# graphdeco-inria/hierarchical-3d-gaussians

Measured on NVIDIA H100. Metric: train-step images/sec (fwd+bwd) @1080p, 3M Gaussians, SH-3, higher is better.
Workload: dtype f32

## Files before the change

### hierarchical-3d-gaussians_b200/csrc/common.cuh

```cuda
#pragma once
#include <cuda_runtime.h>
#include <stdint.h>
#include <stdio.h>
#include <stdlib.h>
#include "../../include/h3dgs.h"

namespace h3dgs {

constexpr float kNearPlane = 0.2f;
constexpr float kFovClamp = 1.3f;
constexpr float kDilation = 0.3f;
constexpr float kLambdaFloor = 0.1f;
constexpr int kTile = H3DGS_TILE;
constexpr int kTilePixels = kTile * kTile;
constexpr float kAlphaCap = 0.99f;
constexpr float kAlphaSkip = 1.0f / 255.0f;
constexpr float kTStop = 0.0001f;
constexpr float kWEps = 0.0000001f;
constexpr uint32_t kKidsMask = 0xFFFFFu;
constexpr int kClampShift = 20;
constexpr uint32_t kSortedKidsMask = 0xFFFFu;
constexpr int kBlockShift = 16;

struct __align__(16) Record { float4 a, b, c; };
// ... 43 lines not shown
    } while (0)

#define H3_LAUNCHED(name, debug, stream)                                                   \
    do {                                                                                   \
        h3dgs::g_launches++;                                                               \
        cudaError_t e__ = cudaGetLastError();                                              \
        if (e__ == cudaSuccess && (debug)) e__ = cudaStreamSynchronize(stream);            \
        if (e__ != cudaSuccess) {                                                          \
            h3dgs::set_error("kernel %s failed: %s", name, cudaGetErrorString(e__));       \
            return H3DGS_ECUDA;                                                            \
        }                                                                                  \
    } while (0)

int launch_preprocess(const h3dgs_raster_args& a, int32_t* radii, float* depths, uint32_t* tiles_touched,
                      uint8_t* rank_mask, Record* records, uint32_t* tile_count, ScanInfo* info, cudaStream_t s);
int launch_tile_scan(const h3dgs_raster_args& a, const uint32_t* tile_count, uint32_t* ranges, ScanInfo* info,
                     uint32_t cap_entries, uint32_t cap_list, cudaStream_t s);
int launch_tile_binning(const h3dgs_raster_args& a, const int32_t* radii, const float* depths, const Record* records,
                        int64_t D, uint32_t max_count, uint8_t* bin, const BinLayout& bl, const uint32_t* ranges,
                        const ScanInfo* info, uint32_t* tile_count, cudaStream_t s);
int launch_preprocess_color(const h3dgs_raster_args& a, const int32_t* radii, const uint32_t* tiles_touched,
                            Record* records, cudaStream_t s);
int launch_sh_backward(const h3dgs_raster_args& a, const int32_t* radii, const uint8_t* rank_mask, const Record* records,
                       const float* accum, float* dL_dmeans3D, float* dL_dsh, cudaStream_t s);
int launch_scan(const uint32_t* in, uint32_t* out, int n, void* temp, size_t temp_bytes, cudaStream_t s, bool debug);
size_t scan_temp_bytes(int n);
size_t sort_temp_bytes(int64_t n);
int launch_binning(const h3dgs_raster_args& a, const int32_t* radii, const float* depths, const uint32_t* offsets,
                   const Record* records, int64_t D, uint8_t* bin, const BinLayout& bl, uint32_t* ranges,
                   cudaStream_t s);
int launch_render_forward(const h3dgs_raster_args& a, const uint32_t* ranges, const Record* sorted_records,
                          float* out_color, float* out_invdepth, float* final_T, uint32_t* n_contrib,
                          uint32_t* tile_max_contrib, cudaStream_t s);
int launch_render_backward(const h3dgs_raster_args& a, const uint32_t* ranges, const Record* sorted_records,
                           const uint32_t* point_list, const float* final_T, const uint32_t* n_contrib,
                           const uint32_t* tile_max_contrib, const float* dL_dcolor, const float* dL_dinvdepth,
                           float* accum , cudaStream_t s);
int launch_preprocess_backward(const h3dgs_raster_args& a, const int32_t* radii, const uint8_t* rank_mask, const Record* records,
                               const float* accum, float* dL_dmeans3D, float* dL_dmeans2D, float* dL_dsh,
                               float* dL_dcolors, float* dL_dopacities, float* dL_dscales, float* dL_drots,
                               float* dL_dcov3D, cudaStream_t s);

#ifdef __CUDACC__
__device__ __forceinline__ void quad_pixel(int tile_x, int tile_y, int warp, int lane, int& px, int& py0) {
    px = tile_x * kTile + 8 * (warp & 1) + (lane & 7);
    py0 = tile_y * kTile + 8 * (warp >> 1) + 2 * (lane >> 3);
}

__device__ __forceinline__ void group_pixel(int tile_x, int tile_y, int warp, int lane, int& px, int& py0) {
    const int g = lane >> 3, k = lane & 7;
    px = tile_x * kTile + 8 * (warp & 1) + 4 * (g & 1) + (k & 3);
    py0 = tile_y * kTile + 8 * (warp >> 1) + 4 * (g >> 1) + 2 * (k >> 2);
}
inline bool use_group_walk(bool dflt) {
    const char* e = getenv("H3DGS_GROUPWALK");
    return (e && e[0]) ? e[0] != '0' : dflt;
}

#endif

struct PeerPtrs { void* p[H3DGS_MAX_PEERS]; int n; };
inline PeerPtrs peer_ptrs(void* const* src, int n) {
    PeerPtrs r; r.n = n > 1 ? n : 0;
    for (int k = 0; k < H3DGS_MAX_PEERS; k++) r.p[k] = (k < r.n) ? src[k] : nullptr;
    return r;
}
struct RowCycle { int shift, world, rank; };
inline RowCycle row_cycle(const h3dgs_raster_args& a) {
    RowCycle c; c.world = a.peer_count > 1 ? a.peer_count : 0; c.rank = a.shard_index; c.shift = a.grad_cyclic_log2;
    return c;
}
inline int cyclic_local_rows(const RowCycle& c, int P) {
    const int blocks = (P + (1 << c.shift) - 1) >> c.shift;
    return ((blocks + c.world - 1 - c.rank) / c.world) << c.shift;
}
#ifdef __CUDACC__
__device__ __forceinline__ int cyclic_row(const RowCycle& c, int local) {
    return ((((local >> c.shift) * c.world + c.rank)) << c.shift) + (local & ((1 << c.shift) - 1));
}
__device__ __forceinline__ bool cyclic_owned(const RowCycle& c, int row) { return ((row >> c.shift) % c.world) == c.rank; }
#endif

#ifdef __CUDACC__
struct StagePtrs { const float* own; const float* stage; int n, rank; size_t slot_floats; };
template <int NPAIR>
__device__ __forceinline__ void gather_accum_pairs(const StagePtrs& sp, uint32_t mask, int i, int first, float (&out)[2 * NPAIR]) {
#pragma unroll
    for (int k = 0; k < 2 * NPAIR; k++) out[k] = 0.f;
#pragma unroll
    for (int r = 0; r < H3DGS_MAX_PEERS; r++) {
        if (r < sp.n && ((mask >> r) & 1u)) {
            const float* row = (r == sp.rank ? sp.own : sp.stage + (size_t)r * sp.slot_floats) + (size_t)i * 10 + 2 * first;
#pragma unroll
            for (int k = 0; k < NPAIR; k++) {
                const float2 v = __ldcg(reinterpret_cast<const float2*>(row + 2 * k));
                out[2 * k] += v.x; out[2 * k + 1] += v.y;
            }
        }
    }
}
#endif
inline StagePtrs stage_ptrs(const h3dgs_raster_args& a, const float* accum) {
    StagePtrs sp; sp.own = accum; sp.n = a.peer_count > 1 ? a.peer_count : 0; sp.rank = a.shard_index;
    sp.stage = sp.n ? static_cast<const float*>(a.peer_stage[a.shard_index]) : nullptr;
    sp.slot_floats = (size_t)a.P * 10;
    return sp;
// ... 18 lines not shown
```

### hierarchical-3d-gaussians_b200/csrc/pair_math.cuh

```cuda
#pragma once

#ifdef H3_PAIR_HOST_EMU
#include <math.h>
#include <stdint.h>
#define H3_PM_FN static inline
namespace h3dgs {
#ifndef H3_SIMT_EMU
struct float4 { float x, y, z, w; };
constexpr float kAlphaCap = 0.99f;
constexpr float kAlphaSkip = 1.0f / 255.0f;
constexpr float kTStop = 0.0001f;
constexpr uint32_t kSortedKidsMask = 0xFFFFu;
#endif
struct f2 { float lo, hi; };
H3_PM_FN f2 pk(float lo, float hi) { return f2{lo, hi}; }
H3_PM_FN void upk(f2 v, float& lo, float& hi) { lo = v.lo; hi = v.hi; }
H3_PM_FN f2 fma2(f2 a, f2 b, f2 c) { return f2{fmaf(a.lo, b.lo, c.lo), fmaf(a.hi, b.hi, c.hi)}; }
H3_PM_FN f2 mul2(f2 a, f2 b) { return f2{a.lo * b.lo, a.hi * b.hi}; }
H3_PM_FN f2 add2(f2 a, f2 b) { return f2{a.lo + b.lo, a.hi + b.hi}; }
H3_PM_FN f2 sub2(f2 a, f2 b) { return f2{a.lo - b.lo, a.hi - b.hi}; }
H3_PM_FN float fast_exp2(float x) { return exp2f(x); }
H3_PM_FN float fast_log2(float x) { return log2f(x); }
H3_PM_FN float rcp_approx(float x) { return 1.0f / x; }
H3_PM_FN float rsq_approx(float x) { return 1.0f / sqrtf(x); }
#else
#define H3_PM_FN __device__ __forceinline__
namespace h3dgs {
struct f2 { float lo, hi; };
H3_PM_FN f2 pk(float lo, float hi) { return f2{lo, hi}; }
H3_PM_FN void upk(f2 v, float& lo, float& hi) { lo = v.lo; hi = v.hi; }
H3_PM_FN f2 fma2(f2 a, f2 b, f2 c) { return f2{__fmaf_rn(a.lo, b.lo, c.lo), __fmaf_rn(a.hi, b.hi, c.hi)}; }
H3_PM_FN f2 mul2(f2 a, f2 b) { return f2{__fmul_rn(a.lo, b.lo), __fmul_rn(a.hi, b.hi)}; }
H3_PM_FN f2 add2(f2 a, f2 b) { return f2{__fadd_rn(a.lo, b.lo), __fadd_rn(a.hi, b.hi)}; }
H3_PM_FN f2 sub2(f2 a, f2 b) { return f2{__fsub_rn(a.lo, b.lo), __fsub_rn(a.hi, b.hi)}; }
H3_PM_FN float fast_exp2(float x) { float y; asm("ex2.approx.ftz.f32 %0, %1;" : "=f"(y) : "f"(x)); return y; }
H3_PM_FN float fast_log2(float x) { float y; asm("lg2.approx.ftz.f32 %0, %1;" : "=f"(y) : "f"(x)); return y; }
H3_PM_FN float rcp_approx(float x) { float y; asm("rcp.approx.ftz.f32 %0, %1;" : "=f"(y) : "f"(x)); return y; }
H3_PM_FN float rsq_approx(float x) { float y; asm("rsqrt.approx.ftz.f32 %0, %1;" : "=f"(y) : "f"(x)); return y; }
#endif

H3_PM_FN f2 bc(float x) { return pk(x, x); }
H3_PM_FN float lo(f2 v) { float a, b; upk(v, a, b); return a; }
H3_PM_FN float hi(f2 v) { float a, b; upk(v, a, b); return b; }
H3_PM_FN float hsum(f2 v) { float a, b; upk(v, a, b); return a + b; }
H3_PM_FN f2 sel2(bool p0, bool p1, f2 x, f2 y) {
    float x0, x1, y0, y1; upk(x, x0, x1); upk(y, y0, y1);
    return pk(p0 ? x0 : y0, p1 ? x1 : y1);
}
H3_PM_FN f2 ex2_2(f2 v) { float a, b; upk(v, a, b); return pk(fast_exp2(a), fast_exp2(b)); }
H3_PM_FN float fast_rcp(float x) { const float r = rcp_approx(x); return r * (2.0f - x * r); }
H3_PM_FN f2 rcp2(f2 x) {
    float x0, x1; upk(x, x0, x1);
    const f2 r = pk(rcp_approx(x0), rcp_approx(x1));
    return mul2(r, fma2(pk(-x0, -x1), r, bc(2.0f)));
}

H3_PM_FN f2 pair_power(const float4& a, const float4& bb, float dx, f2 nfpy, f2& d) {
    d = add2(bc(a.y), nfpy);
    const float A = (a.z * dx) * (dx * -0.5f), B = -a.w * dx, C = -0.5f * bb.x;
    return fma2(fma2(bc(C), d, bc(B)), d, bc(A));
}
H3_PM_FN void pair_gauss(f2 power, float opacity, f2& G, f2& abase) {
    G = ex2_2(mul2(power, bc(1.4426950408889634f)));
    float a0, a1; upk(mul2(bc(opacity), G), a0, a1);
    abase = pk(fminf(kAlphaCap, a0), fminf(kAlphaCap, a1));
}
template <bool HIER, bool GRAD>
H3_PM_FN void pair_hier_alpha(f2 a, float t, uint32_t k , f2& alpha, f2& dadb) {
    alpha = a; dadb = bc(1.0f);
    if (!HIER) return;
    if (k <= 1u || t >= 1.0f) return;
    const float u = 1.0f - t;
    float a0, a1; upk(a, a0, a1);
    float o0, o1; upk(sub2(bc(1.0f), a), o0, o1);
    if (k == 2u) {
        const f2 r = pk(rsq_approx(o0), rsq_approx(o1));
        const f2 s = mul2(pk(o0, o1), r);
        f2 S = fma2(a, bc(0.02734375f), bc(0.0390625f));
        S = fma2(a, S, bc(0.0625f));
        S = fma2(a, S, bc(0.125f));
        S = fma2(a, S, bc(0.5f));
        const f2 omr = sel2(a0 < 0.0625f, a1 < 0.0625f, mul2(a, S), sub2(bc(1.0f), s));
        alpha = fma2(bc(u), omr, mul2(bc(t), a));
        if (GRAD) dadb = fma2(bc(0.5f * u), r, bc(t));
        return;
    }
    const float ik = fast_rcp((float)k);
    const f2 l2 = pk(fast_log2(o0), fast_log2(o1));
    f2 L = fma2(a, bc(0.2f), bc(0.25f));
    L = fma2(a, L, bc(0.33333334f));
    L = fma2(a, L, bc(0.5f));
    L = fma2(a, L, bc(1.0f));
    const f2 yn = sel2(a0 < 0.0625f, a1 < 0.0625f, mul2(mul2(a, L), bc(ik)), mul2(l2, bc(-0.6931472f * ik)));
    f2 S = fma2(yn, bc(-0.041666668f), bc(0.16666667f));
    S = fma2(yn, S, bc(-0.5f));
    S = fma2(yn, S, bc(1.0f));
    const f2 omr_series = mul2(yn, S);
    const f2 omr_mufu = sub2(bc(1.0f), ex2_2(mul2(l2, bc(ik))));
    float y0, y1; upk(yn, y0, y1);
    const f2 omr = sel2(y0 < 0.0625f, y1 < 0.0625f, omr_series, omr_mufu);
    alpha = fma2(bc(u), omr, mul2(bc(t), a));
    if (GRAD) dadb = fma2(bc(u * ik), ex2_2(mul2(l2, bc(ik - 1.0f))), bc(t));
}

H3_PM_FN f2 pair_blend(f2 pw, f2 al, f2& T, bool& done0, bool& done1, bool& v0, bool& v1, bool active = true) {
    const f2 tT = mul2(T, sub2(bc(1.0f), al));
    float pw0, pw1, al0, al1, tT0, tT1;
    upk(pw, pw0, pw1); upk(al, al0, al1); upk(tT, tT0, tT1);
    v0 = active && !done0 && pw0 <= 0.0f && al0 >= kAlphaSkip;
    v1 = active && !done1 && pw1 <= 0.0f && al1 >= kAlphaSkip;
    if (v0 && tT0 < kTStop) { done0 = true; v0 = false; }
    if (v1 && tT1 < kTStop) { done1 = true; v1 = false; }
    const f2 w = sel2(v0, v1, mul2(al, T), bc(0.f));
    T = sel2(v0, v1, tT, T);
    return w;
}

struct PairState { f2 T, acc; };

template <bool HIER, bool DEPTH>
H3_PM_FN void pair_grad(const float4& a, const float4& bb, float dx, f2 d, f2 G, f2 alpha, f2 dadb, f2 cg, f2 T_final,
                        f2 neg_bg_dot, f2 g0, f2 g1, f2 g2, f2 gd, PairState& st, float (&v)[10])
{
    const f2 rcp = rcp2(sub2(bc(1.0f), alpha));
    const f2 diff = sub2(cg, st.acc);
    const f2 dL_dalpha = mul2(fma2(st.T, diff, mul2(T_final, neg_bg_dot)), rcp);
    const f2 dL_dab = HIER ? mul2(dL_dalpha, dadb) : dL_dalpha;
    st.T = mul2(st.T, rcp);
    const f2 w = mul2(alpha, st.T);
    st.acc = fma2(alpha, diff, st.acc);
    float p0, p1, d0, d1;
    upk(mul2(G, dL_dab), p0, p1);
    upk(d, d0, d1);
    const float dp0 = d0 * p0, dp1 = d1 * p1;
    const float S0 = p0 + p1, S1 = dp0 + dp1, S2 = fmaf(d0, dp0, d1 * dp1);
    const float oS0 = bb.y * S0, oS1 = bb.y * S1, dxoS0 = dx * oS0;
    v[0] = fmaf(-a.w, oS1, -a.z * dxoS0);
    v[1] = fmaf(-a.w, dxoS0, -bb.x * oS1);
    v[2] = dx * dxoS0;
    v[3] = dx * oS1;
    v[4] = bb.y * S2;
    v[5] = S0;
    float w0, w1;
    upk(w, w0, w1);
    v[6] = fmaf(w0, lo(g0), w1 * hi(g0)); v[7] = fmaf(w0, lo(g1), w1 * hi(g1)); v[8] = fmaf(w0, lo(g2), w1 * hi(g2));
    if (DEPTH) v[9] = fmaf(w0, lo(gd), w1 * hi(gd));
}

}
#undef H3_PM_FN
```

### hierarchical-3d-gaussians_b200/csrc/render_backward.cu

```cuda
#include "common.cuh"
#include "tma.cuh"

namespace h3dgs {

#ifdef H3_BLEND_OCC8
constexpr int kBwdBatch = 224;
constexpr int kBwdMinBlocks = 8;
#else
constexpr int kBwdBatch = 256;
constexpr int kBwdMinBlocks = 1;
#endif
constexpr int kBwdStages = 2;

__device__ __forceinline__ float xchg_add(float keep, float send, int mask) {
    return keep + __shfl_xor_sync(0xffffffffu, send, mask);
}
template <int SPAN, bool DEPTH>
__device__ __forceinline__ float span_reduce(const float (&v)[10], int lane, float& x) {
    constexpr int top = SPAN / 2, mid = SPAN / 4, low = SPAN / 8;
    const bool bt = lane & top, bm = lane & mid, bl = lane & low;
    float a[4], b[2];
#pragma unroll
    for (int i = 0; i < 4; i++) a[i] = xchg_add(bt ? v[5 + i] : v[i], bt ? v[i] : v[5 + i], top);
    x = DEPTH ? xchg_add(bt ? v[9] : v[4], bt ? v[4] : v[9], top) : xchg_add(v[4], v[4], top);
#pragma unroll
    for (int i = 0; i < 2; i++) b[i] = xchg_add(bm ? a[2 + i] : a[i], bm ? a[i] : a[2 + i], mid);
    x = xchg_add(x, x, mid);
    float r = xchg_add(bl ? b[1] : b[0], bl ? b[0] : b[1], low);
    x = xchg_add(x, x, low);
#pragma unroll
    for (int m = low / 2; m >= 1; m /= 2) { r = xchg_add(r, r, m); x = xchg_add(x, x, m); }
    return r;
}
template <int SPAN>
__device__ __forceinline__ int span_slot(int k) { const int q = k / (SPAN / 8); return q < 4 ? q : q + 1; }

constexpr int kBwdThreads = 128;

template <bool HIER, bool DEPTH, bool GROUPS>
__global__ void __launch_bounds__(kBwdThreads, kBwdMinBlocks)
render_backward_kernel(int W, int H, int gx, int shard_count, int shard_index, const uint2* __restrict__ ranges,
                       const Record* __restrict__ sorted, const uint32_t* __restrict__ point_list,
                       const float* __restrict__ bg, const float* __restrict__ final_T,
                       const uint32_t* __restrict__ n_contrib, const uint32_t* __restrict__ tile_max_contrib,
                       const float* __restrict__ dL_dcolor, const float* __restrict__ dL_dinvdepth,
                       float* __restrict__ accum)
{
    __shared__ __align__(128) Record s_rec[kBwdStages][kBwdBatch];
    __shared__ uint32_t s_id[kBwdStages][kBwdBatch];
    __shared__ __align__(8) uint64_t s_full[kBwdStages];
    __shared__ __align__(16) uint8_t s_list[GROUPS ? kBwdThreads / 32 : 1][4][GROUPS ? kBwdBatch : 4];

    const int tid = threadIdx.x, lane = tid & 31, warp = tid >> 5;
    const int tile_x = blockIdx.x % gx;
    const int tile_y = (blockIdx.x / gx) * shard_count + shard_index;
    const int tile = tile_y * gx + tile_x;
    const uint2 range = ranges[tile];
    const int n = min((int)(range.y - range.x), (int)tile_max_contrib[tile]);
    const int nb = (n + kBwdBatch - 1) / kBwdBatch;
    if (nb == 0) return;
    const Record* src = sorted + range.x;
    const uint32_t* ids = point_list + range.x;

    auto stage_ids = [&](int it) {
        const int b = nb - 1 - it, st = it % kBwdStages;
        for (int k = tid; k < kBwdBatch; k += kBwdThreads) {
            const int e = b * kBwdBatch + k;
            if (e < n) s_id[st][k] = ids[e];
        }
    };
    for (int it = 0; it < kBwdStages && it < nb; it++) stage_ids(it);
    if (GROUPS)
        for (int k = lane; k < kBwdBatch; k += 32) reinterpret_cast<uint32_t*>(&s_list[warp][0][0])[k] = 0u;
    if (tid == 0) {
        for (int s = 0; s < kBwdStages; s++) mbar_init(&s_full[s], 1);
        fence_mbar_init();
    }
    __syncthreads();
    auto issue = [&](int it) {
        const int b = nb - 1 - it, st = it % kBwdStages;
        const uint32_t bytes = (uint32_t)min(kBwdBatch, n - b * kBwdBatch) * (uint32_t)sizeof(Record);
        mbar_arrive_expect_tx(&s_full[st], bytes);
        tma_load_1d(&s_rec[st][0], src + (size_t)b * kBwdBatch, bytes, &s_full[st]);
    };
    if (tid == 0)
        for (int it = 0; it < kBwdStages && it < nb; it++) issue(it);

    int px, py0;
    if (GROUPS) group_pixel(tile_x, tile_y, warp, lane, px, py0);
    else quad_pixel(tile_x, tile_y, warp, lane, px, py0);
    const int k8 = lane & 7;
    const int slot = GROUPS ? span_slot<8>(k8)
                            : (lane & 3) == 0 ? span_slot<32>(lane) : lane == 1 ? 4 : (DEPTH && lane == 17) ? 9 : -1;
    const int xslot = k8 == 0 ? 4 : (DEPTH && k8 == 4) ? 9 : -1;
    const int grp = lane >> 3;
    const int py1 = py0 + 1;
    const bool in0 = px < W && py0 < H, in1 = px < W && py1 < H;
    const float fpx = (float)px;
    const f2 nfpy = pk(-(float)py0, -(float)py1);
    const size_t pix0 = (size_t)py0 * W + px, pix1 = (size_t)py1 * W + px, plane = (size_t)H * W;
    const float Tf0 = in0 ? final_T[pix0] : 0.f, Tf1 = in1 ? final_T[pix1] : 0.f;
    const f2 Tf = pk(Tf0, Tf1);
    PairState ps = {Tf, bc(0.f)};
    const int last0 = in0 ? (int)n_contrib[pix0] : 0, last1 = in1 ? (int)n_contrib[pix1] : 0;
    float ga0 = 0.f, ga1 = 0.f, ga2 = 0.f, gad = 0.f, gb0 = 0.f, gb1 = 0.f, gb2 = 0.f, gbd = 0.f;
    if (in0) { ga0 = dL_dcolor[pix0]; ga1 = dL_dcolor[plane + pix0]; ga2 = dL_dcolor[2 * plane + pix0]; if (DEPTH) gad = dL_dinvdepth[pix0]; }
    if (in1) { gb0 = dL_dcolor[pix1]; gb1 = dL_dcolor[plane + pix1]; gb2 = dL_dcolor[2 * plane + pix1]; if (DEPTH) gbd = dL_dinvdepth[pix1]; }
    const f2 g0 = pk(ga0, gb0), g1 = pk(ga1, gb1), g2 = pk(ga2, gb2), gd = pk(gad, gbd);
    const f2 neg_bgd = pk(-(bg[0] * ga0 + bg[1] * ga1 + bg[2] * ga2), -(bg[0] * gb0 + bg[1] * gb1 + bg[2] * gb2));
    const int wlast = (int)__reduce_max_sync(0xffffffffu, (unsigned)max(last0, last1));
    const int qsel = kBlockShift + 4 * warp;
    int gl0, gl1, gl2, gl3;
    {
        int gm = max(last0, last1);
        gm = max(gm, __shfl_xor_sync(0xffffffffu, gm, 4)); gm = max(gm, __shfl_xor_sync(0xffffffffu, gm, 2));
        gm = max(gm, __shfl_xor_sync(0xffffffffu, gm, 1));
        gl0 = __shfl_sync(0xffffffffu, gm, 0); gl1 = __shfl_sync(0xffffffffu, gm, 8);
        gl2 = __shfl_sync(0xffffffffu, gm, 16); gl3 = __shfl_sync(0xffffffffu, gm, 24);
    }

    for (int it = 0; it < nb; it++) {
        const int st = it % kBwdStages, b = nb - 1 - it;
        mbar_wait(&s_full[st], (uint32_t)((it / kBwdStages) & 1));
        const int cnt = min(kBwdBatch, n - b * kBwdBatch);
        const Record* rec = &s_rec[st][0];
        auto replay_entry = [&](int j, bool has) {
            const int e = b * kBwdBatch + j;
            const float4 a = rec[j].a;
            const float4 bb = rec[j].b;
            const uint32_t gid = s_id[st][j];
            const uint32_t kb = __float_as_uint(bb.w);
            const float dx = a.x - fpx;
            f2 d, G, al, dadb = bc(1.0f);
            const f2 pw = pair_power(a, bb, dx, nfpy, d);
            pair_gauss(pw, bb.y, G, al);
            float pw0, pw1, al0, al1;
            upk(pw, pw0, pw1); upk(al, al0, al1);
            bool v0 = has && e < last0 && pw0 <= 0.0f && al0 >= kAlphaSkip;
            bool v1 = has && e < last1 && pw1 <= 0.0f && al1 >= kAlphaSkip;
            if (lane == 0) H3_STAT(0, 1);
            if ((lane & 7) == 0 && has) H3_STAT(3, 1);
            if (!__any_sync(0xffffffffu, v0 || v1)) { if (lane == 0) H3_STAT(1, 1); return; }
            if (HIER) {
                pair_hier_alpha<HIER, true>(al, bb.z, kb & kSortedKidsMask, al, dadb);
                upk(al, al0, al1);
                v0 = v0 && al0 >= kAlphaSkip;
                v1 = v1 && al1 >= kAlphaSkip;
            }
            H3_STAT(2, (v0 ? 1 : 0) + (v1 ? 1 : 0));
#ifdef H3_SIMT_EMU
            { const uint32_t tk = __ballot_sync(0xffffffffu, v0 || v1);
              if (GROUPS && (lane & 7) == 0 && has && ((tk >> (8 * grp)) & 0xFFu) == 0u) H3_STAT(4, 1); }
#endif
            G = sel2(v0, v1, G, bc(0.f));
            al = sel2(v0, v1, al, bc(0.f));
            const float4 c = rec[j].c;
            f2 cg = fma2(bc(c.z), g2, fma2(bc(c.y), g1, mul2(bc(c.x), g0)));
            if (DEPTH) cg = fma2(bc(c.w), gd, cg);
            float v[10];
            pair_grad<HIER, DEPTH>(a, bb, dx, d, G, al, dadb, cg, Tf, neg_bgd, g0, g1, g2, gd, ps, v);
            float* row = accum + (size_t)gid * kAccum;
            float x;
            if (GROUPS) {
                const bool taker = ((__ballot_sync(0xffffffffu, v0 || v1) >> (8 * grp)) & 0xFFu) != 0u;
                const float r = span_reduce<8, DEPTH>(v, lane, x);
                if (taker) atomicAdd(row + slot, r);
                if (taker && xslot >= 0) atomicAdd(row + xslot, x);
            } else {
                const float r = span_reduce<32, DEPTH>(v, lane, x);
                if (slot >= 0) atomicAdd(row + slot, (lane & 3) == 0 ? r : x);
            }
        };
        if (GROUPS) {
            uint8_t* lst = &s_list[warp][0][0];
            const uint32_t lt = (1u << lane) - 1u;
            int c0 = 0, c1 = 0, c2 = 0, c3 = 0;
            for (int j0 = 0; j0 < cnt; j0 += 32) {
                const int jl = j0 + lane, e = b * kBwdBatch + jl;
                uint32_t nib = jl < cnt ? (__float_as_uint(rec[jl].b.w) >> qsel) & 0xFu : 0u;
                nib &= (e < gl0 ? 1u : 0u) | (e < gl1 ? 2u : 0u) | (e < gl2 ? 4u : 0u) | (e < gl3 ? 8u : 0u);
                const uint32_t m0 = __ballot_sync(0xffffffffu, nib & 1u), m1 = __ballot_sync(0xffffffffu, nib & 2u);
                const uint32_t m2 = __ballot_sync(0xffffffffu, nib & 4u), m3 = __ballot_sync(0xffffffffu, nib & 8u);
                if (nib & 1u) lst[c0 + __popc(m0 & lt)] = (uint8_t)jl;
                if (nib & 2u) lst[kBwdBatch + c1 + __popc(m1 & lt)] = (uint8_t)jl;
                if (nib & 4u) lst[2 * kBwdBatch + c2 + __popc(m2 & lt)] = (uint8_t)jl;
                if (nib & 8u) lst[3 * kBwdBatch + c3 + __popc(m3 & lt)] = (uint8_t)jl;
                c0 += __popc(m0); c1 += __popc(m1); c2 += __popc(m2); c3 += __popc(m3);
            }
            __syncwarp();
            const int mylen = grp == 0 ? c0 : grp == 1 ? c1 : grp == 2 ? c2 : c3;
            const int maxlen = max(max(c0, c1), max(c2, c3));
            const uint8_t* my = lst + grp * kBwdBatch;
            for (int i = maxlen - 1; i >= 0; i--) replay_entry((int)my[i], i < mylen);
            __syncwarp();
        } else {
            for (int j0 = (cnt - 1) & ~31; j0 >= 0; j0 -= 32) {
                const int jl = j0 + lane;
                const uint32_t nib = (jl < cnt && (b * kBwdBatch + jl) < wlast) ? (__float_as_uint(rec[jl].b.w) >> qsel) & 0xFu : 0u;
                uint32_t m = __ballot_sync(0xffffffffu, nib != 0u);
                while (m != 0u) {
                    const int top = 31 - __clz(m);
                    m &= ~(1u << top);
                    replay_entry(j0 + top, true);
                }
            }
        }
        __syncthreads();
        if (it + kBwdStages < nb) {
            if (tid == 0) issue(it + kBwdStages);
            stage_ids(it + kBwdStages);
        }
    }
}

int launch_render_backward(const h3dgs_raster_args& a, const uint32_t* ranges, const Record* sorted_records,
                           const uint32_t* point_list, const float* final_T, const uint32_t* n_contrib,
                           const uint32_t* tile_max_contrib, const float* dL_dcolor, const float* dL_dinvdepth,
                           float* accum, cudaStream_t s)
{
    const int W = a.image_width, H = a.image_height;
    const int gx = (W + kTile - 1) / kTile, gy = (H + kTile - 1) / kTile;
    const int sc = a.shard_count > 0 ? a.shard_count : 1, si = a.shard_count > 0 ? a.shard_index : 0;
    const int rows = (gy + sc - 1 - si) / sc;
    if (rows <= 0 || gx <= 0) return H3DGS_OK;
    const bool hier = a.interpolation_weights != nullptr;
    const bool depth = a.do_depth != 0 && dL_dinvdepth != nullptr;
    const dim3 grid(gx * rows), block(kBwdThreads);
    ProfScope prof(H3DGS_STAGE_RENDER_BWD, s);
    const bool groups = use_group_walk(true);
#define LAUNCH(HI, DE, GR)                                                                                          \
    render_backward_kernel<HI, DE, GR><<<grid, block, 0, s>>>(W, H, gx, sc, si, (const uint2*)ranges, sorted_records, \
                                                              point_list, a.bg, final_T, n_contrib, tile_max_contrib, \
                                                              dL_dcolor, dL_dinvdepth, accum)
#define LAUNCH2(HI, DE) do { if (groups) LAUNCH(HI, DE, true); else LAUNCH(HI, DE, false); } while (0)
    if (hier) { if (depth) LAUNCH2(true, true); else LAUNCH2(true, false); }
    else      { if (depth) LAUNCH2(false, true); else LAUNCH2(false, false); }
#undef LAUNCH2
#undef LAUNCH
    H3_LAUNCHED("render_backward", a.debug, s);
    return H3DGS_OK;
}

}
```

### hierarchical-3d-gaussians_b200/csrc/render_forward.cu

```cuda
#include "common.cuh"
#include "tma.cuh"

namespace h3dgs {

#ifdef H3_BLEND_OCC8
constexpr int kFwdBatch = 224;
constexpr int kFwdMinBlocks = 8;
#else
constexpr int kFwdBatch = 256;
constexpr int kFwdMinBlocks = 1;
#endif
constexpr int kFwdStages = 2;

constexpr int kFwdThreads = 128;

template <bool HIER, bool DEPTH, bool GROUPS>
__global__ void __launch_bounds__(kFwdThreads, kFwdMinBlocks)
render_forward_kernel(int W, int H, int gx, int shard_count, int shard_index, const uint2* __restrict__ ranges,
                      const Record* __restrict__ sorted, const float* __restrict__ bg, float* __restrict__ out_color,
                      float* __restrict__ out_invdepth, float* __restrict__ final_T, uint32_t* __restrict__ n_contrib,
                      uint32_t* __restrict__ tile_max_contrib, const PeerPtrs peers)
{
    __shared__ __align__(128) Record s_rec[kFwdStages][kFwdBatch];
    __shared__ __align__(8) uint64_t s_full[kFwdStages];
    __shared__ uint32_t s_max;
    __shared__ uint8_t s_list[GROUPS ? kFwdThreads / 32 : 1][4][GROUPS ? kFwdBatch : 4];

    const int tid = threadIdx.x, warp = tid >> 5, lane = tid & 31;
    const int tile_x = blockIdx.x % gx;
    const int tile_y = (blockIdx.x / gx) * shard_count + shard_index;
    const int tile = tile_y * gx + tile_x;
    const uint2 range = ranges[tile];
    const int n = (int)(range.y - range.x);
    const int nb = (n + kFwdBatch - 1) / kFwdBatch;
    const Record* src = sorted + range.x;

    if (tid == 0) {
        for (int s = 0; s < kFwdStages; s++) mbar_init(&s_full[s], 1);
        s_max = 0;
        fence_mbar_init();
    }
    __syncthreads();
    int issued = 0;
    if (tid == 0) {
        for (int s = 0; s < kFwdStages && s < nb; s++) {
            const uint32_t bytes = (uint32_t)min(kFwdBatch, n - s * kFwdBatch) * (uint32_t)sizeof(Record);
            mbar_arrive_expect_tx(&s_full[s], bytes);
            tma_load_1d(&s_rec[s][0], src + (size_t)s * kFwdBatch, bytes, &s_full[s]);
        }
    }
    issued = min(kFwdStages, nb);

    int px, py0;
    if (GROUPS) group_pixel(tile_x, tile_y, warp, lane, px, py0);
    else quad_pixel(tile_x, tile_y, warp, lane, px, py0);
    const int py1 = py0 + 1;
    const bool in0 = px < W && py0 < H, in1 = px < W && py1 < H;
    const float fpx = (float)px;
    const f2 nfpy = pk(-(float)py0, -(float)py1);
    bool done0 = !in0, done1 = !in1;
    f2 T = bc(1.0f);
    float Ca0 = 0.f, Ca1 = 0.f, Ca2 = 0.f, Cb0 = 0.f, Cb1 = 0.f, Cb2 = 0.f, inv0 = 0.f, inv1 = 0.f;
    uint32_t last0 = 0, last1 = 0;
    const int qsel = kBlockShift + 4 * warp;
    const int grp = lane >> 3;

    int waited = 0;
    for (int b = 0; b < nb; b++) {
        const int st = b % kFwdStages;
        mbar_wait(&s_full[st], (uint32_t)((b / kFwdStages) & 1));
// ... 149 lines not shown
```

Before: 342.8.

## Render backward with 64-thread blocks, four pixels per thread, 8 sub-groups

Restructures the backward rasterization kernel so each thread handles a column of four pixels (two packed pairs) instead of two. Blocks shrink to 64 threads with eight 4-lane groups per warp, and each group walks its own compacted list of Gaussians. The cross-lane reduction becomes a short 2-step shuffle feeding vectorized float2 atomics, and the batch size drops to 192 with a min-blocks hint of 9. The aim is fewer shuffles and atomics per pixel, plus finer-grained culling per sub-group. The cost is more registers per thread, and per-entry work is wasted when only part of a four-pixel column is covered.

```diff
diff --git a/hierarchical-3d-gaussians_b200/csrc/common.cuh b/hierarchical-3d-gaussians_b200/csrc/common.cuh
--- a/hierarchical-3d-gaussians_b200/csrc/common.cuh
+++ b/hierarchical-3d-gaussians_b200/csrc/common.cuh
@@ -119,6 +119,11 @@
     px = tile_x * kTile + 8 * (warp & 1) + 4 * (g & 1) + (k & 3);
     py0 = tile_y * kTile + 8 * (warp >> 1) + 4 * (g >> 1) + 2 * (k >> 2);
 }
+__device__ __forceinline__ void column_pixel(int tile_x, int tile_y, int warp, int lane, int& px, int& py0) {
+    const int g = lane >> 2, k = lane & 3;
+    px = tile_x * kTile + 8 * (g >> 2) + 4 * (g & 1) + k;
+    py0 = tile_y * kTile + 8 * warp + 4 * ((g >> 1) & 1);
+}
 inline bool use_group_walk(bool dflt) {
     const char* e = getenv("H3DGS_GROUPWALK");
     return (e && e[0]) ? e[0] != '0' : dflt;
diff --git a/hierarchical-3d-gaussians_b200/csrc/pair_math.cuh b/hierarchical-3d-gaussians_b200/csrc/pair_math.cuh
--- a/hierarchical-3d-gaussians_b200/csrc/pair_math.cuh
+++ b/hierarchical-3d-gaussians_b200/csrc/pair_math.cuh
@@ -65,27 +65,26 @@
     float a0, a1; upk(mul2(bc(opacity), G), a0, a1);
     abase = pk(fminf(kAlphaCap, a0), fminf(kAlphaCap, a1));
 }
-template <bool HIER, bool GRAD>
-H3_PM_FN void pair_hier_alpha(f2 a, float t, uint32_t k , f2& alpha, f2& dadb) {
-    alpha = a; dadb = bc(1.0f);
-    if (!HIER) return;
-    if (k <= 1u || t >= 1.0f) return;
+template <bool GRAD>
+H3_PM_FN void pair_hier_k2(f2 a, float t, f2& alpha, f2& dadb) {
     const float u = 1.0f - t;
     float a0, a1; upk(a, a0, a1);
     float o0, o1; upk(sub2(bc(1.0f), a), o0, o1);
-    if (k == 2u) {
-        const f2 r = pk(rsq_approx(o0), rsq_approx(o1));
-        const f2 s = mul2(pk(o0, o1), r);
-        f2 S = fma2(a, bc(0.02734375f), bc(0.0390625f));
-        S = fma2(a, S, bc(0.0625f));
-        S = fma2(a, S, bc(0.125f));
-        S = fma2(a, S, bc(0.5f));
-        const f2 omr = sel2(a0 < 0.0625f, a1 < 0.0625f, mul2(a, S), sub2(bc(1.0f), s));
-        alpha = fma2(bc(u), omr, mul2(bc(t), a));
-        if (GRAD) dadb = fma2(bc(0.5f * u), r, bc(t));
-        return;
-    }
-    const float ik = fast_rcp((float)k);
+    const f2 r = pk(rsq_approx(o0), rsq_approx(o1));
+    const f2 s = mul2(pk(o0, o1), r);
+    f2 S = fma2(a, bc(0.02734375f), bc(0.0390625f));
+    S = fma2(a, S, bc(0.0625f));
+    S = fma2(a, S, bc(0.125f));
+    S = fma2(a, S, bc(0.5f));
+    const f2 omr = sel2(a0 < 0.0625f, a1 < 0.0625f, mul2(a, S), sub2(bc(1.0f), s));
+    alpha = fma2(bc(u), omr, mul2(bc(t), a));
+    if (GRAD) dadb = fma2(bc(0.5f * u), r, bc(t));
+}
+template <bool GRAD>
+H3_PM_FN void pair_hier_kn(f2 a, float t, float ik, f2& alpha, f2& dadb) {
+    const float u = 1.0f - t;
+    float a0, a1; upk(a, a0, a1);
+    float o0, o1; upk(sub2(bc(1.0f), a), o0, o1);
     const f2 l2 = pk(fast_log2(o0), fast_log2(o1));
     f2 L = fma2(a, bc(0.2f), bc(0.25f));
     L = fma2(a, L, bc(0.33333334f));
@@ -102,6 +101,14 @@
     alpha = fma2(bc(u), omr, mul2(bc(t), a));
     if (GRAD) dadb = fma2(bc(u * ik), ex2_2(mul2(l2, bc(ik - 1.0f))), bc(t));
 }
+template <bool HIER, bool GRAD>
+H3_PM_FN void pair_hier_alpha(f2 a, float t, uint32_t k , f2& alpha, f2& dadb) {
+    alpha = a; dadb = bc(1.0f);
+    if (!HIER) return;
+    if (k <= 1u || t >= 1.0f) return;
+    if (k == 2u) { pair_hier_k2<GRAD>(a, t, alpha, dadb); return; }
+    pair_hier_kn<GRAD>(a, t, fast_rcp((float)k), alpha, dadb);
+}
 
 H3_PM_FN f2 pair_blend(f2 pw, f2 al, f2& T, bool& done0, bool& done1, bool& v0, bool& v1, bool active = true) {
     const f2 tT = mul2(T, sub2(bc(1.0f), al));
@@ -118,9 +125,10 @@
 
 struct PairState { f2 T, acc; };
 
+struct EntrySums { float S0, S1, S2, c[4]; };
 template <bool HIER, bool DEPTH>
-H3_PM_FN void pair_grad(const float4& a, const float4& bb, float dx, f2 d, f2 G, f2 alpha, f2 dadb, f2 cg, f2 T_final,
-                        f2 neg_bg_dot, f2 g0, f2 g1, f2 g2, f2 gd, PairState& st, float (&v)[10])
+H3_PM_FN EntrySums pair_sums(f2 d, f2 G, f2 alpha, f2 dadb, f2 cg, f2 T_final, f2 neg_bg_dot, f2 g0, f2 g1, f2 g2, f2 gd,
+                             PairState& st)
 {
     const f2 rcp = rcp2(sub2(bc(1.0f), alpha));
     const f2 diff = sub2(cg, st.acc);
@@ -133,18 +141,71 @@
     upk(mul2(G, dL_dab), p0, p1);
     upk(d, d0, d1);
     const float dp0 = d0 * p0, dp1 = d1 * p1;
-    const float S0 = p0 + p1, S1 = dp0 + dp1, S2 = fmaf(d0, dp0, d1 * dp1);
-    const float oS0 = bb.y * S0, oS1 = bb.y * S1, dxoS0 = dx * oS0;
+    EntrySums s;
+    s.S0 = p0 + p1; s.S1 = dp0 + dp1; s.S2 = fmaf(d0, dp0, d1 * dp1);
+    float w0, w1;
+    upk(w, w0, w1);
+    s.c[0] = fmaf(w0, lo(g0), w1 * hi(g0)); s.c[1] = fmaf(w0, lo(g1), w1 * hi(g1)); s.c[2] = fmaf(w0, lo(g2), w1 * hi(g2));
+    s.c[3] = DEPTH ? fmaf(w0, lo(gd), w1 * hi(gd)) : 0.0f;
+    return s;
+}
+template <bool DEPTH>
+H3_PM_FN void entry_grad(const float4& a, const float4& bb, float dx, const EntrySums& s, float (&v)[10]) {
+    const float oS0 = bb.y * s.S0, oS1 = bb.y * s.S1, dxoS0 = dx * oS0;
     v[0] = fmaf(-a.w, oS1, -a.z * dxoS0);
     v[1] = fmaf(-a.w, dxoS0, -bb.x * oS1);
     v[2] = dx * dxoS0;
     v[3] = dx * oS1;
-    v[4] = bb.y * S2;
-    v[5] = S0;
-    float w0, w1;
-    upk(w, w0, w1);
-    v[6] = fmaf(w0, lo(g0), w1 * hi(g0)); v[7] = fmaf(w0, lo(g1), w1 * hi(g1)); v[8] = fmaf(w0, lo(g2), w1 * hi(g2));
-    if (DEPTH) v[9] = fmaf(w0, lo(gd), w1 * hi(gd));
+    v[4] = bb.y * s.S2;
+    v[5] = s.S0;
+    v[6] = s.c[0]; v[7] = s.c[1]; v[8] = s.c[2];
+    if (DEPTH) v[9] = s.c[3];
+}
+template <bool HIER, bool DEPTH>
+H3_PM_FN void pair_grad(const float4& a, const float4& bb, float dx, f2 d, f2 G, f2 alpha, f2 dadb, f2 cg, f2 T_final,
+                        f2 neg_bg_dot, f2 g0, f2 g1, f2 g2, f2 gd, PairState& st, float (&v)[10])
+{
+    entry_grad<DEPTH>(a, bb, dx, pair_sums<HIER, DEPTH>(d, G, alpha, dadb, cg, T_final, neg_bg_dot, g0, g1, g2, gd, st), v);
+}
+
+struct f2x2 { f2 p0, p1; };
+H3_PM_FN f2x2 quad_power(const float4& a, const float4& bb, float dx, const f2x2& nfpy, f2x2& d) {
+    f2x2 pw;
+    pw.p0 = pair_power(a, bb, dx, nfpy.p0, d.p0);
+    pw.p1 = pair_power(a, bb, dx, nfpy.p1, d.p1);
+    return pw;
+}
+H3_PM_FN void quad_gauss(const f2x2& power, float opacity, f2x2& G, f2x2& abase) {
+    pair_gauss(power.p0, opacity, G.p0, abase.p0);
+    pair_gauss(power.p1, opacity, G.p1, abase.p1);
+}
+template <bool HIER, bool GRAD>
+H3_PM_FN void quad_hier_alpha(f2x2 a, float t, uint32_t k, f2x2& alpha, f2x2& dadb) {
+    alpha = a; dadb.p0 = dadb.p1 = bc(1.0f);
+    if (!HIER) return;
+    if (k <= 1u || t >= 1.0f) return;
+    if (k == 2u) {
+        pair_hier_k2<GRAD>(a.p0, t, alpha.p0, dadb.p0);
+        pair_hier_k2<GRAD>(a.p1, t, alpha.p1, dadb.p1);
+        return;
+    }
+    const float ik = fast_rcp((float)k);
+    pair_hier_kn<GRAD>(a.p0, t, ik, alpha.p0, dadb.p0);
+    pair_hier_kn<GRAD>(a.p1, t, ik, alpha.p1, dadb.p1);
+}
+template <bool HIER, bool DEPTH>
+H3_PM_FN void quad_grad(const float4& a, const float4& bb, float dx, const f2x2& d, const f2x2& G, const f2x2& alpha,
+                        const f2x2& dadb, const f2x2& cg, const f2x2& T_final, const f2x2& neg_bg_dot, const f2x2& g0,
+                        const f2x2& g1, const f2x2& g2, const f2x2& gd, PairState (&st)[2], float (&v)[10])
+{
+    const EntrySums s0 = pair_sums<HIER, DEPTH>(d.p0, G.p0, alpha.p0, dadb.p0, cg.p0, T_final.p0, neg_bg_dot.p0,
+                                                g0.p0, g1.p0, g2.p0, gd.p0, st[0]);
+    const EntrySums s1 = pair_sums<HIER, DEPTH>(d.p1, G.p1, alpha.p1, dadb.p1, cg.p1, T_final.p1, neg_bg_dot.p1,
+                                                g0.p1, g1.p1, g2.p1, gd.p1, st[1]);
+    EntrySums s;
+    s.S0 = s0.S0 + s1.S0; s.S1 = s0.S1 + s1.S1; s.S2 = s0.S2 + s1.S2;
+    for (int i = 0; i < 4; i++) s.c[i] = s0.c[i] + s1.c[i];
+    entry_grad<DEPTH>(a, bb, dx, s, v);
 }
 
 }
diff --git a/hierarchical-3d-gaussians_b200/csrc/render_backward.cu b/hierarchical-3d-gaussians_b200/csrc/render_backward.cu
--- a/hierarchical-3d-gaussians_b200/csrc/render_backward.cu
+++ b/hierarchical-3d-gaussians_b200/csrc/render_backward.cu
@@ -3,42 +3,35 @@
 
 namespace h3dgs {
 
-#ifdef H3_BLEND_OCC8
-constexpr int kBwdBatch = 224;
-constexpr int kBwdMinBlocks = 8;
-#else
-constexpr int kBwdBatch = 256;
-constexpr int kBwdMinBlocks = 1;
-#endif
+constexpr int kBwdBatch = 192;
 constexpr int kBwdStages = 2;
+constexpr int kBwdThreads = 64;
+constexpr int kBwdGroups = 8;
 
 __device__ __forceinline__ float xchg_add(float keep, float send, int mask) {
     return keep + __shfl_xor_sync(0xffffffffu, send, mask);
 }
-template <int SPAN, bool DEPTH>
-__device__ __forceinline__ float span_reduce(const float (&v)[10], int lane, float& x) {
-    constexpr int top = SPAN / 2, mid = SPAN / 4, low = SPAN / 8;
-    const bool bt = lane & top, bm = lane & mid, bl = lane & low;
-    float a[4], b[2];
-#pragma unroll
-    for (int i = 0; i < 4; i++) a[i] = xchg_add(bt ? v[5 + i] : v[i], bt ? v[i] : v[5 + i], top);
-    x = DEPTH ? xchg_add(bt ? v[9] : v[4], bt ? v[4] : v[9], top) : xchg_add(v[4], v[4], top);
-#pragma unroll
-    for (int i = 0; i < 2; i++) b[i] = xchg_add(bm ? a[2 + i] : a[i], bm ? a[i] : a[2 + i], mid);
-    x = xchg_add(x, x, mid);
-    float r = xchg_add(bl ? b[1] : b[0], bl ? b[0] : b[1], low);
-    x = xchg_add(x, x, low);
-#pragma unroll
-    for (int m = low / 2; m >= 1; m /= 2) { r = xchg_add(r, r, m); x = xchg_add(x, x, m); }
-    return r;
-}
-template <int SPAN>
-__device__ __forceinline__ int span_slot(int k) { const int q = k / (SPAN / 8); return q < 4 ? q : q + 1; }
-
-constexpr int kBwdThreads = 128;
-
-template <bool HIER, bool DEPTH, bool GROUPS>
-__global__ void __launch_bounds__(kBwdThreads, kBwdMinBlocks)
+template <bool DEPTH>
+__device__ __forceinline__ void group_reduce(const float (&v)[10], int lane, float& r0, float& r1, float& x) {
+    const bool b1 = lane & 2, b0 = lane & 1;
+    float a[4];
+#pragma unroll
+    for (int i = 0; i < 4; i++) a[i] = xchg_add(b1 ? v[4 + i] : v[i], b1 ? v[i] : v[4 + i], 2);
+    x = DEPTH ? xchg_add(b1 ? v[9] : v[8], b1 ? v[8] : v[9], 2) : xchg_add(v[8], v[8], 2);
+    r0 = xchg_add(b0 ? a[2] : a[0], b0 ? a[0] : a[2], 1);
+    r1 = xchg_add(b0 ? a[3] : a[1], b0 ? a[1] : a[3], 1);
+    x = xchg_add(x, x, 1);
+}
+__device__ __forceinline__ void red_add2(float* p, float x, float y) {
+#ifdef H3_SIMT_EMU
+    atomicAdd(p, x); atomicAdd(p + 1, y);
+#else
+    atomicAdd(reinterpret_cast<float2*>(p), make_float2(x, y));
+#endif
+}
+
+template <bool HIER, bool DEPTH>
+__global__ void __launch_bounds__(kBwdThreads, 9)
 render_backward_kernel(int W, int H, int gx, int shard_count, int shard_index, const uint2* __restrict__ ranges,
                        const Record* __restrict__ sorted, const uint32_t* __restrict__ point_list,
                        const float* __restrict__ bg, const float* __restrict__ final_T,
@@ -49,7 +42,7 @@
     __shared__ __align__(128) Record s_rec[kBwdStages][kBwdBatch];
     __shared__ uint32_t s_id[kBwdStages][kBwdBatch];
     __shared__ __align__(8) uint64_t s_full[kBwdStages];
-    __shared__ __align__(16) uint8_t s_list[GROUPS ? kBwdThreads / 32 : 1][4][GROUPS ? kBwdBatch : 4];
+    __shared__ __align__(16) uint8_t s_list[kBwdThreads / 32][kBwdGroups][kBwdBatch];
 
     const int tid = threadIdx.x, lane = tid & 31, warp = tid >> 5;
     const int tile_x = blockIdx.x % gx;
@@ -70,8 +63,7 @@
         }
     };
     for (int it = 0; it < kBwdStages && it < nb; it++) stage_ids(it);
-    if (GROUPS)
-        for (int k = lane; k < kBwdBatch; k += 32) reinterpret_cast<uint32_t*>(&s_list[warp][0][0])[k] = 0u;
+    for (int k = lane; k < kBwdGroups * kBwdBatch / 4; k += 32) reinterpret_cast<uint32_t*>(&s_list[warp][0][0])[k] = 0u;
     if (tid == 0) {
         for (int s = 0; s < kBwdStages; s++) mbar_init(&s_full[s], 1);
         fence_mbar_init();
@@ -87,36 +79,34 @@
         for (int it = 0; it < kBwdStages && it < nb; it++) issue(it);
 
     int px, py0;
-    if (GROUPS) group_pixel(tile_x, tile_y, warp, lane, px, py0);
-    else quad_pixel(tile_x, tile_y, warp, lane, px, py0);
-    const int k8 = lane & 7;
-    const int slot = GROUPS ? span_slot<8>(k8)
-                            : (lane & 3) == 0 ? span_slot<32>(lane) : lane == 1 ? 4 : (DEPTH && lane == 17) ? 9 : -1;
-    const int xslot = k8 == 0 ? 4 : (DEPTH && k8 == 4) ? 9 : -1;
-    const int grp = lane >> 3;
-    const int py1 = py0 + 1;
-    const bool in0 = px < W && py0 < H, in1 = px < W && py1 < H;
+    column_pixel(tile_x, tile_y, warp, lane, px, py0);
+    const int grp = lane >> 2, k4 = lane & 3;
     const float fpx = (float)px;
-    const f2 nfpy = pk(-(float)py0, -(float)py1);
-    const size_t pix0 = (size_t)py0 * W + px, pix1 = (size_t)py1 * W + px, plane = (size_t)H * W;
-    const float Tf0 = in0 ? final_T[pix0] : 0.f, Tf1 = in1 ? final_T[pix1] : 0.f;
-    const f2 Tf = pk(Tf0, Tf1);
-    PairState ps = {Tf, bc(0.f)};
-    const int last0 = in0 ? (int)n_contrib[pix0] : 0, last1 = in1 ? (int)n_contrib[pix1] : 0;
-    float ga0 = 0.f, ga1 = 0.f, ga2 = 0.f, gad = 0.f, gb0 = 0.f, gb1 = 0.f, gb2 = 0.f, gbd = 0.f;
-    if (in0) { ga0 = dL_dcolor[pix0]; ga1 = dL_dcolor[plane + pix0]; ga2 = dL_dcolor[2 * plane + pix0]; if (DEPTH) gad = dL_dinvdepth[pix0]; }
-    if (in1) { gb0 = dL_dcolor[pix1]; gb1 = dL_dcolor[plane + pix1]; gb2 = dL_dcolor[2 * plane + pix1]; if (DEPTH) gbd = dL_dinvdepth[pix1]; }
-    const f2 g0 = pk(ga0, gb0), g1 = pk(ga1, gb1), g2 = pk(ga2, gb2), gd = pk(gad, gbd);
-    const f2 neg_bgd = pk(-(bg[0] * ga0 + bg[1] * ga1 + bg[2] * ga2), -(bg[0] * gb0 + bg[1] * gb1 + bg[2] * gb2));
-    const int wlast = (int)__reduce_max_sync(0xffffffffu, (unsigned)max(last0, last1));
-    const int qsel = kBlockShift + 4 * warp;
-    int gl0, gl1, gl2, gl3;
+    const f2x2 nfpy = {pk(-(float)py0, -(float)(py0 + 1)), pk(-(float)(py0 + 2), -(float)(py0 + 3))};
+    const size_t plane = (size_t)H * W;
+    float Tf[4], gc[4][4], nbg[4];
+    int last[4];
+#pragma unroll
+    for (int i = 0; i < 4; i++) {
+        const bool in = px < W && py0 + i < H;
+        const size_t pix = (size_t)(py0 + i) * W + px;
+        Tf[i] = in ? final_T[pix] : 0.f;
+        last[i] = in ? (int)n_contrib[pix] : 0;
+#pragma unroll
+        for (int ch = 0; ch < 3; ch++) gc[ch][i] = in ? dL_dcolor[ch * plane + pix] : 0.f;
+        gc[3][i] = (DEPTH && in) ? dL_dinvdepth[pix] : 0.f;
+        nbg[i] = -(bg[0] * gc[0][i] + bg[1] * gc[1][i] + bg[2] * gc[2][i]);
+    }
+    auto quad = [](const float (&x)[4]) { return f2x2{pk(x[0], x[1]), pk(x[2], x[3])}; };
+    const f2x2 Tfq = quad(Tf), g0 = quad(gc[0]), g1 = quad(gc[1]), g2 = quad(gc[2]), gd = quad(gc[3]), neg_bgd = quad(nbg);
+    PairState ps[2] = {{Tfq.p0, bc(0.f)}, {Tfq.p1, bc(0.f)}};
+    const int qsel = kBlockShift + 8 * warp;
+    int gl[kBwdGroups];
     {
-        int gm = max(last0, last1);
-        gm = max(gm, __shfl_xor_sync(0xffffffffu, gm, 4)); gm = max(gm, __shfl_xor_sync(0xffffffffu, gm, 2));
-        gm = max(gm, __shfl_xor_sync(0xffffffffu, gm, 1));
-        gl0 = __shfl_sync(0xffffffffu, gm, 0); gl1 = __shfl_sync(0xffffffffu, gm, 8);
-        gl2 = __shfl_sync(0xffffffffu, gm, 16); gl3 = __shfl_sync(0xffffffffu, gm, 24);
+        int gm = max(max(last[0], last[1]), max(last[2], last[3]));
+        gm = max(gm, __shfl_xor_sync(0xffffffffu, gm, 2)); gm = max(gm, __shfl_xor_sync(0xffffffffu, gm, 1));
+#pragma unroll
+        for (int g = 0; g < kBwdGroups; g++) gl[g] = __shfl_sync(0xffffffffu, gm, 4 * g);
     }
 
     for (int it = 0; it < nb; it++) {
@@ -131,80 +121,71 @@
             const uint32_t gid = s_id[st][j];
             const uint32_t kb = __float_as_uint(bb.w);
             const float dx = a.x - fpx;
-            f2 d, G, al, dadb = bc(1.0f);
-            const f2 pw = pair_power(a, bb, dx, nfpy, d);
-            pair_gauss(pw, bb.y, G, al);
-            float pw0, pw1, al0, al1;
-            upk(pw, pw0, pw1); upk(al, al0, al1);
-            bool v0 = has && e < last0 && pw0 <= 0.0f && al0 >= kAlphaSkip;
-            bool v1 = has && e < last1 && pw1 <= 0.0f && al1 >= kAlphaSkip;
+            f2x2 d, G, al, dadb = {bc(1.0f), bc(1.0f)};
+            const f2x2 pw = quad_power(a, bb, dx, nfpy, d);
+            quad_gauss(pw, bb.y, G, al);
+            float pwv[4], alv[4];
+            upk(pw.p0, pwv[0], pwv[1]); upk(pw.p1, pwv[2], pwv[3]);
+            upk(al.p0, alv[0], alv[1]); upk(al.p1, alv[2], alv[3]);
+            bool v[4];
+#pragma unroll
+            for (int i = 0; i < 4; i++) v[i] = has && e < last[i] && pwv[i] <= 0.0f && alv[i] >= kAlphaSkip;
             if (lane == 0) H3_STAT(0, 1);
-            if ((lane & 7) == 0 && has) H3_STAT(3, 1);
-            if (!__any_sync(0xffffffffu, v0 || v1)) { if (lane == 0) H3_STAT(1, 1); return; }
+            if (k4 == 0 && has) H3_STAT(3, 1);
+            if (!__any_sync(0xffffffffu, v[0] || v[1] || v[2] || v[3])) { if (lane == 0) H3_STAT(1, 1); return; }
             if (HIER) {
-                pair_hier_alpha<HIER, true>(al, bb.z, kb & kSortedKidsMask, al, dadb);
-                upk(al, al0, al1);
-                v0 = v0 && al0 >= kAlphaSkip;
-                v1 = v1 && al1 >= kAlphaSkip;
+                quad_hier_alpha<HIER, true>(al, bb.z, kb & kSortedKidsMask, al, dadb);
+                upk(al.p0, alv[0], alv[1]); upk(al.p1, alv[2], alv[3]);
+#pragma unroll
+                for (int i = 0; i < 4; i++) v[i] = v[i] && alv[i] >= kAlphaSkip;
             }
-            H3_STAT(2, (v0 ? 1 : 0) + (v1 ? 1 : 0));
+            H3_STAT(2, (v[0] ? 1 : 0) + (v[1] ? 1 : 0) + (v[2] ? 1 : 0) + (v[3] ? 1 : 0));
+            const uint32_t tk = __ballot_sync(0xffffffffu, v[0] || v[1] || v[2] || v[3]);
+            const bool taker = ((tk >> (4 * grp)) & 0xFu) != 0u;
 #ifdef H3_SIMT_EMU
-            { const uint32_t tk = __ballot_sync(0xffffffffu, v0 || v1);
-              if (GROUPS && (lane & 7) == 0 && has && ((tk >> (8 * grp)) & 0xFFu) == 0u) H3_STAT(4, 1); }
+            if (k4 == 0 && has && !taker) H3_STAT(4, 1);
 #endif
-            G = sel2(v0, v1, G, bc(0.f));
-            al = sel2(v0, v1, al, bc(0.f));
+            G.p0 = sel2(v[0], v[1], G.p0, bc(0.f)); G.p1 = sel2(v[2], v[3], G.p1, bc(0.f));
+            al.p0 = sel2(v[0], v[1], al.p0, bc(0.f)); al.p1 = sel2(v[2], v[3], al.p1, bc(0.f));
             const float4 c = rec[j].c;
-            f2 cg = fma2(bc(c.z), g2, fma2(bc(c.y), g1, mul2(bc(c.x), g0)));
-            if (DEPTH) cg = fma2(bc(c.w), gd, cg);
-            float v[10];
-            pair_grad<HIER, DEPTH>(a, bb, dx, d, G, al, dadb, cg, Tf, neg_bgd, g0, g1, g2, gd, ps, v);
+            f2x2 cg;
+            cg.p0 = fma2(bc(c.z), g2.p0, fma2(bc(c.y), g1.p0, mul2(bc(c.x), g0.p0)));
+            cg.p1 = fma2(bc(c.z), g2.p1, fma2(bc(c.y), g1.p1, mul2(bc(c.x), g0.p1)));
+            if (DEPTH) { cg.p0 = fma2(bc(c.w), gd.p0, cg.p0); cg.p1 = fma2(bc(c.w), gd.p1, cg.p1); }
+            float vs[10];
+            quad_grad<HIER, DEPTH>(a, bb, dx, d, G, al, dadb, cg, Tfq, neg_bgd, g0, g1, g2, gd, ps, vs);
+            float r0, r1, x;
+            group_reduce<DEPTH>(vs, lane, r0, r1, x);
             float* row = accum + (size_t)gid * kAccum;
-            float x;
-            if (GROUPS) {
-                const bool taker = ((__ballot_sync(0xffffffffu, v0 || v1) >> (8 * grp)) & 0xFFu) != 0u;
-                const float r = span_reduce<8, DEPTH>(v, lane, x);
-                if (taker) atomicAdd(row + slot, r);
-                if (taker && xslot >= 0) atomicAdd(row + xslot, x);
-            } else {
-                const float r = span_reduce<32, DEPTH>(v, lane, x);
-                if (slot >= 0) atomicAdd(row + slot, (lane & 3) == 0 ? r : x);
-            }
+            if (taker) red_add2(row + 2 * k4, r0, r1);
+            if (taker && (k4 == 0 || (DEPTH && k4 == 2))) atomicAdd(row + 8 + (k4 >> 1), x);
         };
-        if (GROUPS) {
-            uint8_t* lst = &s_list[warp][0][0];
-            const uint32_t lt = (1u << lane) - 1u;
-            int c0 = 0, c1 = 0, c2 = 0, c3 = 0;
-            for (int j0 = 0; j0 < cnt; j0 += 32) {
-                const int jl = j0 + lane, e = b * kBwdBatch + jl;
-                uint32_t nib = jl < cnt ? (__float_as_uint(rec[jl].b.w) >> qsel) & 0xFu : 0u;
-                nib &= (e < gl0 ? 1u : 0u) | (e < gl1 ? 2u : 0u) | (e < gl2 ? 4u : 0u) | (e < gl3 ? 8u : 0u);
-                const uint32_t m0 = __ballot_sync(0xffffffffu, nib & 1u), m1 = __ballot_sync(0xffffffffu, nib & 2u);
-                const uint32_t m2 = __ballot_sync(0xffffffffu, nib & 4u), m3 = __ballot_sync(0xffffffffu, nib & 8u);
-                if (nib & 1u) lst[c0 + __popc(m0 & lt)] = (uint8_t)jl;
-                if (nib & 2u) lst[kBwdBatch + c1 + __popc(m1 & lt)] = (uint8_t)jl;
-                if (nib & 4u) lst[2 * kBwdBatch + c2 + __popc(m2 & lt)] = (uint8_t)jl;
-                if (nib & 8u) lst[3 * kBwdBatch + c3 + __popc(m3 & lt)] = (uint8_t)jl;
-                c0 += __popc(m0); c1 += __popc(m1); c2 += __popc(m2); c3 += __popc(m3);
-            }
-            __syncwarp();
-            const int mylen = grp == 0 ? c0 : grp == 1 ? c1 : grp == 2 ? c2 : c3;
-            const int maxlen = max(max(c0, c1), max(c2, c3));
-            const uint8_t* my = lst + grp * kBwdBatch;
-            for (int i = maxlen - 1; i >= 0; i--) replay_entry((int)my[i], i < mylen);
-            __syncwarp();
-        } else {
-            for (int j0 = (cnt - 1) & ~31; j0 >= 0; j0 -= 32) {
-                const int jl = j0 + lane;
-                const uint32_t nib = (jl < cnt && (b * kBwdBatch + jl) < wlast) ? (__float_as_uint(rec[jl].b.w) >> qsel) & 0xFu : 0u;
-                uint32_t m = __ballot_sync(0xffffffffu, nib != 0u);
-                while (m != 0u) {
-                    const int top = 31 - __clz(m);
-                    m &= ~(1u << top);
-                    replay_entry(j0 + top, true);
-                }
+        uint8_t* lst = &s_list[warp][0][0];
+        const uint32_t lt = (1u << lane) - 1u;
+        int c[kBwdGroups];
+#pragma unroll
+        for (int g = 0; g < kBwdGroups; g++) c[g] = 0;
+        for (int j0 = 0; j0 < cnt; j0 += 32) {
+            const int jl = j0 + lane, e = b * kBwdBatch + jl;
+            uint32_t bits = jl < cnt ? (__float_as_uint(rec[jl].b.w) >> qsel) & 0xFFu : 0u;
+            uint32_t live = 0u;
+#pragma unroll
+            for (int g = 0; g < kBwdGroups; g++) live |= e < gl[g] ? 1u << g : 0u;
+            bits &= live;
+#pragma unroll
+            for (int g = 0; g < kBwdGroups; g++) {
+                const uint32_t m = __ballot_sync(0xffffffffu, bits & (1u << g));
+                if (bits & (1u << g)) lst[g * kBwdBatch + c[g] + __popc(m & lt)] = (uint8_t)jl;
+                c[g] += __popc(m);
             }
         }
+        __syncwarp();
+        int mylen = 0, maxlen = 0;
+#pragma unroll
+        for (int g = 0; g < kBwdGroups; g++) { mylen = grp == g ? c[g] : mylen; maxlen = max(maxlen, c[g]); }
+        const uint8_t* my = lst + grp * kBwdBatch;
+        for (int i = maxlen - 1; i >= 0; i--) replay_entry((int)my[i], i < mylen);
+        __syncwarp();
         __syncthreads();
         if (it + kBwdStages < nb) {
             if (tid == 0) issue(it + kBwdStages);
@@ -227,15 +208,12 @@
     const bool depth = a.do_depth != 0 && dL_dinvdepth != nullptr;
     const dim3 grid(gx * rows), block(kBwdThreads);
     ProfScope prof(H3DGS_STAGE_RENDER_BWD, s);
-    const bool groups = use_group_walk(true);
-#define LAUNCH(HI, DE, GR)                                                                                          \
-    render_backward_kernel<HI, DE, GR><<<grid, block, 0, s>>>(W, H, gx, sc, si, (const uint2*)ranges, sorted_records, \
-                                                              point_list, a.bg, final_T, n_contrib, tile_max_contrib, \
-                                                              dL_dcolor, dL_dinvdepth, accum)
-#define LAUNCH2(HI, DE) do { if (groups) LAUNCH(HI, DE, true); else LAUNCH(HI, DE, false); } while (0)
-    if (hier) { if (depth) LAUNCH2(true, true); else LAUNCH2(true, false); }
-    else      { if (depth) LAUNCH2(false, true); else LAUNCH2(false, false); }
-#undef LAUNCH2
+#define LAUNCH(HI, DE)                                                                                          \
+    render_backward_kernel<HI, DE><<<grid, block, 0, s>>>(W, H, gx, sc, si, (const uint2*)ranges, sorted_records,   \
+                                                          point_list, a.bg, final_T, n_contrib, tile_max_contrib,   \
+                                                          dL_dcolor, dL_dinvdepth, accum)
+    if (hier) { if (depth) LAUNCH(true, true); else LAUNCH(true, false); }
+    else      { if (depth) LAUNCH(false, true); else LAUNCH(false, false); }
 #undef LAUNCH
     H3_LAUNCHED("render_backward", a.debug, s);
     return H3DGS_OK;
diff --git a/hierarchical-3d-gaussians_b200/csrc/render_forward.cu b/hierarchical-3d-gaussians_b200/csrc/render_forward.cu
--- a/hierarchical-3d-gaussians_b200/csrc/render_forward.cu
+++ b/hierarchical-3d-gaussians_b200/csrc/render_forward.cu
@@ -3,19 +3,13 @@
 
 namespace h3dgs {
 
-#ifdef H3_BLEND_OCC8
-constexpr int kFwdBatch = 224;
-constexpr int kFwdMinBlocks = 8;
-#else
 constexpr int kFwdBatch = 256;
-constexpr int kFwdMinBlocks = 1;
-#endif
 constexpr int kFwdStages = 2;
 
 constexpr int kFwdThreads = 128;
 
 template <bool HIER, bool DEPTH, bool GROUPS>
-__global__ void __launch_bounds__(kFwdThreads, kFwdMinBlocks)
+__global__ void __launch_bounds__(kFwdThreads, 1)
 render_forward_kernel(int W, int H, int gx, int shard_count, int shard_index, const uint2* __restrict__ ranges,
                       const Record* __restrict__ sorted, const float* __restrict__ bg, float* __restrict__ out_color,
                       float* __restrict__ out_invdepth, float* __restrict__ final_T, uint32_t* __restrict__ n_contrib,
```

New measurement: 356.4, median of 6. 1.04x the previous value.
